# CognitiveAISystems/pogema

Hardware: AMD Instinct MI355X
Metric: agent-steps/sec (whole node), 64-agent 64x64 grid, batch=8192 envs (higher is better)
Workload: dtype u32

## Files before the change

include/pogema_amd.h:

```cpp
#ifndef POGEMA_AMD_H
#define POGEMA_AMD_H

#include <stddef.h>
#include <stdint.h>

#ifdef __cplusplus
extern "C" {
#endif

#define PGX_ABI_VERSION 6

#define PGX_OK 0
#define PGX_E_INVALID (-1)
#define PGX_E_HIP (-2)
#define PGX_E_NOMEM (-3)
#define PGX_E_STATE (-4)
#define PGX_E_PLACEMENT (-5)

#define PGX_COLLISION_PRIORITY 0
#define PGX_COLLISION_BLOCK_BOTH 1
#define PGX_COLLISION_SOFT 2

#define PGX_ON_TARGET_FINISH 0
#define PGX_ON_TARGET_RESTART 1
// ... 53 lines not shown

int pgx_create(const pgx_config* cfg, int device, pgx_env** out);
int pgx_destroy(pgx_env* env);
int pgx_check_config(const pgx_config* cfg);

int64_t pgx_obs_elems(const pgx_env* env);
int64_t pgx_agent_elems(const pgx_env* env);

int pgx_reset_from_state(pgx_env* env, const uint8_t* obstacles, const int32_t* agent_xy,
                         const int32_t* target_xy, void* stream);

int pgx_reset_random(pgx_env* env, float density, uint64_t seed, const uint8_t* shared_map,
                     const uint8_t* env_mask, int32_t max_retries, void* stream);

int pgx_regenerate(pgx_env* env, const uint8_t* env_mask, float density, uint64_t seed, const uint8_t* shared_map,
                   int32_t max_retries, void* obs, void* stream);
int64_t pgx_regenerate_failures(pgx_env* env, void* stream);

int pgx_set_map_pool(pgx_env* env, const uint8_t* maps, int32_t num_maps, int32_t* capacity_out, void* stream);
int pgx_reset_pool(pgx_env* env, uint64_t seed, const uint8_t* env_mask, int32_t max_retries, void* stream);
int pgx_regenerate_pool(pgx_env* env, const uint8_t* env_mask, uint64_t seed, int32_t max_retries, void* obs,
                        void* stream);
int pgx_get_map_index(pgx_env* env, int32_t* map_index, void* stream);

int pgx_get_map(pgx_env* env, uint8_t* obstacles, void* stream);

int pgx_step(pgx_env* env, const void* actions, int action_dtype, void* obs, float* rewards,
             uint8_t* terminated, uint8_t* truncated, uint8_t* is_active, void* stream);

int pgx_step_held(pgx_env* env, const void* actions, int action_dtype, void* obs, uint8_t* held, int32_t refresh,
                  float* rewards, uint8_t* terminated, uint8_t* truncated, uint8_t* is_active, void* stream);
int pgx_held_available(const pgx_env* env);

int pgx_xcd_shares(pgx_env* env, int32_t* shares);
int pgx_xcd_tune(pgx_env* env, void* obs, void* obs_alt, int32_t rounds, float* us_equal, float* us_tuned, void* stream);

typedef struct pgx_geometry {
    int32_t lanes_per_env;
    int32_t waves;
    int32_t envs_per_wave;
    int32_t multi_wave;
    int32_t p16;
    int32_t stagger;
    int32_t store_policy;
    int32_t state_stores;
    int32_t grid;
    int32_t lds_bytes;
    int32_t for_rollout;
    int32_t xcd_aware;
} pgx_geometry;
int pgx_get_geometry(const pgx_env* env, int32_t for_rollout, pgx_geometry* out);

typedef struct pgx_rollout_io {
    const void* actions;
    void* obs;
    float* rewards;
    uint8_t* terminated;
    uint8_t* truncated;
    uint8_t* is_active;
    uint8_t* episode_done;
    float* metrics;
    int32_t action_dtype;
    int32_t obs_slots;
    int64_t obs_slot_stride;
    uint64_t policy_seed;
    int64_t policy_step0;
// ... 197 lines not shown
```

pogema_amd/_lib.py:

```python
from __future__ import annotations

import ctypes as C
import os

_HERE = os.path.dirname(os.path.abspath(__file__))
LIB_PATH = os.environ.get("PGX_LIB") or os.path.join(_HERE, "libpogema_amd.so")

PGX_ABI_VERSION = 6

COLLISION_SYSTEMS = {"priority": 0, "block_both": 1, "soft": 2}
ON_TARGET = {"finish": 0, "restart": 1, "nothing": 2}
ACTION_DTYPES = {"int8": 0, "int32": 1, "int64": 2}
SOFT_VERTEX_RULES = {"lowest_index": 0, "all_stay": 1}
SOFT_OCCUPANCY = {"index_order": 0, "exact": 1}
COOP_REWARDS = {"all_solved": 0, "per_agent": 1}
BAD_ACTIONS = {"noop": 0, "flag": 1}
LIFELONG_RNGS = {"build": 0, "numpy": 1}
def _obs_dtypes():
    import torch
    return {torch.float32: 0, torch.uint8: 1, torch.bfloat16: 2, torch.float16: 3}


def obs_elem_bytes(dtype) -> int:
    import torch
# ... 36 lines not shown
PLAN_FIXED_PRIORITY = 1
MAX_WHCA_HORIZON = 31
SWAP_MAX_WALK = 2048
OUTCOMES = ("STAY", "MOVED", "OBSTACLE", "SWAP", "OCCUPIED", "FOLLOW", "CONTESTED")
NUM_OUTCOMES = len(OUTCOMES)
POLICY_CHANNELS = {"obstacles": 0, "agents": 1, "target": 2, "other_goals": 3, "up": 4, "down": 5, "left": 6, "right": 7}
NUM_CHANNELS = len(POLICY_CHANNELS)
COPY_NO_CACHE = 1
DEFAULT_POLICY_CHANNELS = ("obstacles", "agents", "target", "up", "down", "left", "right")
GLOBAL_CHANNELS = {"obstacles": 0, "agents": 1, "targets": 2, "agent_ids": 3, "target_ids": 4}
NUM_GLOBAL_CHANNELS = len(GLOBAL_CHANNELS)
DEFAULT_GLOBAL_CHANNELS = ("obstacles", "agents", "targets")
GLOBAL_ID_CHANNELS = ("agent_ids", "target_ids")
GLOBAL_ID_MAX = {1: 255, 2: 256}
GLOBAL_BAND_CELLS = 8192
TOKEN_CLIP = 20
TOKEN_BLOCKED = 41
TOKEN_ACTION_NONE = 42
TOKEN_ACTION0 = 43
TOKEN_GREEDY0 = 48
TOKEN_PAD = 64
NUM_TOKENS = 65
TOKEN_HISTORY = 5
TOKEN_SLOT_LEN = 10
MAX_TOKEN_SLOTS = 32
MAX_TOKEN_LENGTH = 2048
TOKENS = {"CLIP": TOKEN_CLIP, "BLOCKED": TOKEN_BLOCKED, "ACTION_NONE": TOKEN_ACTION_NONE, "ACTION0": TOKEN_ACTION0,
          "GREEDY0": TOKEN_GREEDY0, "PAD": TOKEN_PAD, "NUM_TOKENS": NUM_TOKENS, "HISTORY": TOKEN_HISTORY,
          "SLOT_LEN": TOKEN_SLOT_LEN, "MAX_SLOTS": MAX_TOKEN_SLOTS, "MAX_LENGTH": MAX_TOKEN_LENGTH}


EXPORTED_SYMBOLS = (
    "pgx_abi_version", "pgx_last_error", "pgx_create", "pgx_check_config", "pgx_destroy", "pgx_obs_elems", "pgx_agent_elems",
    "pgx_reset_from_state", "pgx_reset_random", "pgx_regenerate", "pgx_regenerate_failures", "pgx_get_map", "pgx_step", "pgx_step_held", "pgx_held_available", "pgx_observe", "pgx_set_metrics_buffers", "pgx_get_state", "pgx_generate", "pgx_place_agents",
    "pgx_snapshot_bytes", "pgx_save_snapshot", "pgx_load_snapshot", "pgx_time_observe", "pgx_bad_action_count",
    "pgx_buffers_create", "pgx_buffers_ptr", "pgx_buffers_get_info", "pgx_buffers_destroy", "pgx_set_targets",
    "pgx_np_streams", "pgx_np_streams_host", "pgx_np_generate", "pgx_np_generate_host", "pgx_rollout", "pgx_buffers_stride", "pgx_buffers_drop", "pgx_xcd_shares", "pgx_xcd_tune", "pgx_buffers_create_at", "pgx_time_observe_pair", "pgx_buffers_va_reserved", "pgx_get_geometry",
    "pgx_expert_actions", "pgx_set_map_pool", "pgx_reset_pool", "pgx_regenerate_pool", "pgx_get_map_index",
    "pgx_cost_to_go", "pgx_cost_to_go_bytes", "pgx_cost_to_go_builds", "pgx_visible_agents", "pgx_pibt_actions",
    "pgx_goal_directions", "pgx_shield_actions", "pgx_pibt_plan", "pgx_move_outcomes",
    "pgx_policy_input", "pgx_copy_envs", "pgx_global_state", "pgx_global_state_check",
    "pgx_agent_tokens", "pgx_agent_tokens_length", "pgx_goal_paths", "pgx_pibt_swap_actions", "pgx_pibt_swap_plan",
    "pgx_agent_forecasts", "pgx_blocking", "pgx_path_conflicts", "pgx_whca_plan", "pgx_repair_plan",
)


class PgxError(RuntimeError):
    def __init__(self, code: int, message: str):
        super().__init__(f"pogema_amd engine error {code}: {message}")
        self.code = code


class PgxBuffersInfo(C.Structure):
    _fields_ = [("bytes", C.c_int64), ("count", C.c_int32), ("spread", C.c_int32), ("candidates", C.c_int32),
                ("reserved0", C.c_int32), ("same_zone_us", C.c_float), ("final_us", C.c_float), ("spacer_gib", C.c_double),
                ("buffer_gbs", C.c_float), ("reserved1", C.c_float)]


class PgxGeometry(C.Structure):
    _fields_ = [(n, C.c_int32) for n in ("lanes_per_env", "waves", "envs_per_wave", "multi_wave", "p16", "stagger",
                                          "store_policy", "state_stores", "grid", "lds_bytes", "for_rollout", "xcd_aware")]


class PgxRolloutIO(C.Structure):
    _fields_ = [("actions", C.c_void_p), ("obs", C.c_void_p), ("rewards", C.c_void_p), ("terminated", C.c_void_p),
                ("truncated", C.c_void_p), ("is_active", C.c_void_p), ("episode_done", C.c_void_p), ("metrics", C.c_void_p),
                ("action_dtype", C.c_int32), ("obs_slots", C.c_int32), ("obs_slot_stride", C.c_int64),
# ... 119 lines not shown
    lib.pgx_agent_forecasts.argtypes = [vp, i32, i32, i32, vp, vp, vp]
    lib.pgx_agent_forecasts.restype = C.c_int
    lib.pgx_blocking.argtypes = [vp, i32, i32, vp, vp, vp]
    lib.pgx_blocking.restype = C.c_int
    lib.pgx_path_conflicts.argtypes = [vp, vp, i32, i32, i32, vp, vp, vp, vp, vp]
    lib.pgx_path_conflicts.restype = C.c_int
    lib.pgx_copy_envs.argtypes = [vp, vp, vp, i32, i32, vp]
    lib.pgx_copy_envs.restype = C.c_int
    lib.pgx_set_map_pool.argtypes = [vp, vp, i32, vp, vp]
    lib.pgx_set_map_pool.restype = C.c_int
    lib.pgx_reset_pool.argtypes = [vp, u64, vp, i32, vp]
    lib.pgx_reset_pool.restype = C.c_int
    lib.pgx_regenerate_pool.argtypes = [vp, vp, u64, i32, vp, vp]
    lib.pgx_regenerate_pool.restype = C.c_int
    lib.pgx_get_map_index.argtypes = [vp, vp, vp]
    lib.pgx_get_map_index.restype = C.c_int
    lib.pgx_set_targets.argtypes = [vp, vp, vp, vp]
    lib.pgx_set_targets.restype = C.c_int
    lib.pgx_bad_action_count.argtypes = [vp, vp]
    lib.pgx_bad_action_count.restype = i64
    lib.pgx_time_observe.argtypes = [vp, vp, i32, C.POINTER(C.c_float), vp]
    lib.pgx_time_observe.restype = C.c_int
    lib.pgx_time_observe_pair.argtypes = [vp, vp, vp, i32, C.POINTER(C.c_float), vp]
    lib.pgx_time_observe_pair.restype = C.c_int
    lib.pgx_snapshot_bytes.argtypes = [vp]
    lib.pgx_snapshot_bytes.restype = i64
    lib.pgx_save_snapshot.argtypes = [vp, vp, vp]
    lib.pgx_load_snapshot.argtypes = [vp, vp, vp]
    lib.pgx_save_snapshot.restype = lib.pgx_load_snapshot.restype = C.c_int
    lib.pgx_step.argtypes = [vp, vp, C.c_int, vp, vp, vp, vp, vp, vp]
    lib.pgx_step_held.argtypes = [vp, vp, C.c_int, vp, vp, i32, vp, vp, vp, vp, vp]
    lib.pgx_held_available.argtypes = [vp]
    lib.pgx_step_held.restype = lib.pgx_held_available.restype = C.c_int
    lib.pgx_observe.argtypes = [vp, vp, vp]
    lib.pgx_set_metrics_buffers.argtypes = [vp, vp, vp]
    lib.pgx_get_state.argtypes = [vp, vp, vp, vp, vp, vp, vp]
    lib.pgx_generate.argtypes = [i32, i32, i32, i32, f32, u64, i64, i32, i32, vp, vp, vp]
    lib.pgx_place_agents.argtypes = [i32, i32, i32, i32, u64, i64, i32, i32, vp, i32, vp, vp]
    for name in ("pgx_create", "pgx_destroy", "pgx_reset_from_state", "pgx_reset_random", "pgx_regenerate", "pgx_get_map",
                 "pgx_step", "pgx_observe", "pgx_set_metrics_buffers", "pgx_set_metrics_buffers",
                 "pgx_get_state", "pgx_generate", "pgx_place_agents"):
        getattr(lib, name).restype = C.c_int
    if lib.pgx_abi_version() != PGX_ABI_VERSION:
        raise ImportError(f"{LIB_PATH}: ABI version {lib.pgx_abi_version()} != expected {PGX_ABI_VERSION}; rebuild")
    _lib = lib
    return lib


def check(status: int) -> None:
    if status != 0:
        msg = load().pgx_last_error()
        raise PgxError(status, msg.decode("utf-8", "replace") if msg else "unknown error")
```

pogema_amd/buffers.py:

```python
from __future__ import annotations

import atexit
import collections
import contextlib
import ctypes as C
import os
import threading

import numpy as np
import torch

from . import _lib

_TYPESTR = {torch.float32: "<f4", torch.uint8: "|u1", torch.float16: "<f2", torch.bfloat16: "<f2"}


class _Owner:

    def __init__(self, lib, handle):
        self._lib, self._handle = lib, handle

    def __del__(self):
        try:
            if self._handle is not None and self._handle.value:
# ... 284 lines not shown
            cdata = master.untyped_storage()._cdata
            base = hook(cdata)
            alias = master.detach()
            one = hook(cdata)
            view = alias[2:4].view(torch.int16)
            two = hook(cdata)
            del alias
            still = hook(cdata)
            del view
            back = hook(cdata)
            if not (one == base + 1 and two == base + 2 and still == base + 1 and back == base):
                why = f"torch._C._storage_Use_Count no longer counts tensors per storage ({base}, {one}, {two}, {still}, {back})"
        except Exception as exc:
            why = f"torch._C._storage_Use_Count self-test raised {exc!r}"
    if why is not None:
        import warnings
        warnings.warn(f"pogema_amd: {why} in torch {torch.__version__}; reuse_buffers='recycle' falls back to allocating "
                      f"fresh output tensors per step", RuntimeWarning, stacklevel=2)
        hook = None
    _HOOK = hook
    return hook


_UNSET = object()
_HOOK = _UNSET


class RecyclingOutputs:

    @staticmethod
    def available() -> bool:
        return storage_count_hook() is not None

    def __init__(self, obs_tensors, batch: int, agents: int, zone_ptrs=()):
        if not self.available():
            raise RuntimeError("torch._C._storage_Use_Count is missing or changed its meaning in this torch build")
        self._count = storage_count_hook()
        self._zone_ptrs = frozenset(int(p) for p in zone_ptrs)
        dev = obs_tensors[0].device
        n = batch * agents
        self._sets = []
        for obs in obs_tensors:
            block = torch.empty(n * 7 + 16, dtype=torch.uint8, device=dev)
            members = (obs, block[:4 * n].view(torch.float32).view(batch, agents),
                       block[4 * n:5 * n].view(torch.bool).view(batch, agents),
                       block[5 * n:6 * n].view(torch.bool).view(batch, agents),
                       block[6 * n:7 * n].view(torch.bool).view(batch, agents))
            storages = (obs.untyped_storage(), block.untyped_storage())
            self._sets.append((members, storages, tuple(st._cdata for st in storages)))
        del obs, block, members, storages
        self._idle = [tuple(self._count(c) for c in cdata) for _, _, cdata in self._sets]
        self._held = [torch.full((batch, agents), 255, dtype=torch.uint8, device=dev) for _ in self._sets]
        self._vouched = [None] * len(self._sets)
        self._next = 0
        self.taken = 0
        self.misses = 0

    def __len__(self):
        return len(self._sets)

    def obs_pointers(self):
        return [members[0].data_ptr() for members, _, _ in self._sets]

    def _is_idle(self, i: int) -> bool:
        cdata, idle = self._sets[i][2], self._idle[i]
        return self._count(cdata[0]) == idle[0] and self._count(cdata[1]) == idle[1]

    def free_sets(self) -> int:
        return sum(self._is_idle(i) for i in range(len(self._sets)))

    def retire(self):
        idle = [i for i in range(len(self._sets)) if self._is_idle(i)]
        out = [self._sets[i][0][0] for i in idle if self._sets[i][0][0].data_ptr() in self._zone_ptrs]
        for i in reversed(idle):
            del self._sets[i]
            del self._idle[i]
            del self._held[i]
            del self._vouched[i]
        self._next = 0
        return out

    def _take_index(self):
        n = len(self._sets)
        for k in range(n):
            i = (self._next + k) % n
            if self._is_idle(i):
                self._next = (i + 1) % n
                self.taken += 1
                return i
        self.misses += 1
        return None

    def _hand_out(self, i: int, with_obs: bool):
        m = self._sets[i][0]
        return (m[0].detach() if with_obs else None, m[1].detach(), m[2].detach(), m[3].detach(), m[4].detach())

    @staticmethod
    def _version(t):
        try:
            return t._version
        except Exception:
            return None

    def take(self, with_obs: bool = True):
        i = self._take_index()
        if i is None:
            return None
        if with_obs:
            self._vouched[i] = None
        return self._hand_out(i, with_obs)

    def take_for_step(self, with_obs: bool = True):
        i = self._take_index()
        if i is None:
            return None
        trusted = False
        if with_obs:
            v = self._vouched[i]
            trusted = v is not None and self._version(self._sets[i][0][0]) == v
            self._vouched[i] = None
        return self._hand_out(i, with_obs), self._held[i], trusted, i

    def vouch(self, i: int):
        self._vouched[i] = self._version(self._sets[i][0][0])
```

pogema_amd/csrc/pgx_api.cpp:

```cpp
#include "../../include/pogema_amd.h"

#include <hip/hip_runtime.h>

#include <algorithm>
#include <cstdarg>
#include <cstdio>
#include <cstdlib>
#include <cstring>
#include <new>
#include <string>
#include <vector>

#include "pgx_internal.h"

namespace {
thread_local std::string g_err;
}

namespace pgx {
int fail_msg(int code, const char* fmt, ...) {
    char buf[512];
    va_list ap;
    va_start(ap, fmt);
    vsnprintf(buf, sizeof buf, fmt, ap);
// ... 883 lines not shown
    DeviceGuard guard;
    if (const int rc = enter(guard, e, "pgx_get_map", true)) return rc;
    PGX_HIP(hipMemcpyAsync(obstacles, e->map_u8, (size_t)e->cfg.batch * e->cfg.height * e->cfg.width,
                           hipMemcpyDeviceToDevice, (hipStream_t)stream));
    return PGX_OK;
}

int pgx_step(pgx_env* e, const void* actions, int action_dtype, void* obs, float* rewards, uint8_t* terminated,
             uint8_t* truncated, uint8_t* is_active, void* stream) {
    if (!e || !actions || !rewards || !terminated || !truncated) return fail_msg(PGX_E_INVALID, "pgx_step: null argument");
    if (const int rc = check_action_dtype("pgx_step", action_dtype)) return rc;
    DeviceGuard guard;
    if (const int rc = enter(guard, e, "pgx_step", true)) return rc;
    pgx::StepParams p = step_params(e, e->geo);
    p.mode = pgx::MODE_STEP;
    p.action_dtype = action_dtype;
    p.actions = actions;
    p.obs = static_cast<float*>(obs);
    p.rewards = rewards;
    p.terminated = terminated;
    p.truncated = truncated;
    p.act_out = is_active;
    PGX_HIP(pgx::launch_step(p, e->geo, (hipStream_t)stream));
    return PGX_OK;
}

int pgx_held_available(const pgx_env* e) {
    if (!e) return 0;
    return pgx::held_available(e->geo, e->cfg.num_agents, e->W, obs_elem_bytes(e->cfg.obs_dtype)) ? 1 : 0;
}

int pgx_step_held(pgx_env* e, const void* actions, int action_dtype, void* obs, uint8_t* held, int32_t refresh, float* rewards,
                  uint8_t* terminated, uint8_t* truncated, uint8_t* is_active, void* stream) {
    if (!e || !obs || !held || !pgx_held_available(e))
        return pgx_step(e, actions, action_dtype, obs, rewards, terminated, truncated, is_active, stream);
    if (!actions || !rewards || !terminated || !truncated) return fail_msg(PGX_E_INVALID, "pgx_step_held: null argument");
    if (const int rc = check_action_dtype("pgx_step_held", action_dtype)) return rc;
    DeviceGuard guard;
    if (const int rc = enter(guard, e, "pgx_step_held", true)) return rc;
    pgx::StepParams p = step_params(e, e->geo);
    p.mode = pgx::MODE_STEP;
    p.action_dtype = action_dtype;
    p.actions = actions;
    p.obs = static_cast<float*>(obs);
    p.rewards = rewards;
    p.terminated = terminated;
    p.truncated = truncated;
    p.act_out = is_active;
    PGX_HIP(pgx::launch_step_held(p, e->geo, held, refresh != 0, (hipStream_t)stream));
    return PGX_OK;
}

int pgx_rollout(pgx_env* e, int32_t steps, const pgx_rollout_io* io, void* stream) {
    if (!e || !io || !io->rewards || !io->terminated || !io->truncated)
        return fail_msg(PGX_E_INVALID, "pgx_rollout: null argument");
    if (io->policy_step0 < 0 || io->policy_step0 > ((int64_t)1 << 40))
        return fail_msg(PGX_E_INVALID, "pgx_rollout: policy_step0 outside 0..2^40");
    if (steps < 1) return fail_msg(PGX_E_INVALID, "pgx_rollout: steps must be >= 1, got %d", steps);
    if (const int rc = check_action_dtype("pgx_rollout", io->action_dtype)) return rc;
    if (io->obs && io->obs_slots < 1) return fail_msg(PGX_E_INVALID, "pgx_rollout: obs given but obs_slots = %d", io->obs_slots);
    DeviceGuard guard;
    if (const int rc = enter(guard, e, "pgx_rollout", true)) return rc;
    pgx::StepParams p = step_params(e, e->geo_roll);
    p.mode = pgx::MODE_STEP;
    p.action_dtype = io->action_dtype;
    p.actions = io->actions;
    p.obs = static_cast<float*>(io->obs);
    p.rewards = io->rewards;
    p.terminated = io->terminated;
    p.truncated = io->truncated;
    p.act_out = io->is_active;
    p.metrics_out = io->metrics;
    p.episode_done = io->episode_done;
    const int64_t agents = (int64_t)e->cfg.batch * e->cfg.num_agents;
    const int64_t W = 2 * e->cfg.obs_radius + 1;
    static const int64_t action_bytes[3] = {1, 4, 8};
    pgx::RolloutParams rp;
    rp.steps = steps;
    rp.obs_slots = io->obs ? io->obs_slots : 1;
    rp.resident_bitmap = e->geo_roll.resident_bitmap ? 1 : 0;
    rp.reserved0 = 0;
    rp.actions_stride = agents * action_bytes[io->action_dtype];
// ... 831 lines not shown
```

pogema_amd/csrc/pgx_internal.h:

```cpp
#pragma once
#include <hip/hip_runtime.h>
#include <stddef.h>
#include <stdint.h>

namespace pgx {

int fail_msg(int code, const char* fmt, ...);

#define PGX_HIP(call)                                                                                                      \
    do {                                                                                                                   \
        const hipError_t e__ = (call);                                                                                     \
        if (e__ != hipSuccess)                                                                                             \
            return pgx::fail_msg(PGX_E_HIP, "%s failed: %s (%s:%d)", #call, hipGetErrorString(e__), __FILE__, __LINE__); \
    } while (0)

struct DeviceGuard {
    int prev = -1;
    bool changed = false;
    hipError_t err = hipSuccess;
    DeviceGuard() = default;
    explicit DeviceGuard(int dev) { (void)select(dev); }
    DeviceGuard(const DeviceGuard&) = delete;
    DeviceGuard& operator=(const DeviceGuard&) = delete;
    hipError_t select(int dev) {
// ... 82 lines not shown
    int64_t env_index_base;
    const uint32_t* obst;
    uint32_t* pos;
    uint32_t* tgt;
    uint8_t* active;
    int32_t* elapsed;
    const uint32_t* pos0;
    const uint32_t* tgt0;
    const uint32_t* comp_begin;
    const uint32_t* comp_len;
    const uint32_t* comp_cells;
    uint32_t* tcount;
    NpGen* np_state;
    const NpGen* np_state0;
    int4* macc;
    float* metrics_out;
    uint8_t* episode_done;
    uint32_t* bad_count;
    const void* actions;
    float* obs;
    float* rewards;
    uint8_t* terminated;
    uint8_t* truncated;
    uint8_t* act_out;
    const uint8_t* only;
    unsigned long long* dbg;
};

struct HeldParams {
    uint8_t* held;
    int32_t refresh;
    int32_t lds_word;
    int32_t words;
};

struct RolloutParams {
    int32_t steps;
    int32_t obs_slots;
    int32_t resident_bitmap;
    int32_t reserved0;
    int64_t actions_stride;
    int64_t agents_stride;
    int64_t envs_stride;
    int64_t obs_stride;
    uint64_t policy_seed;
    int64_t policy_step0;
    int8_t* actions_out;
};

struct StepGeometry {
    int G;
    int waves;
    int epw;
    bool multi_wave;
    bool p16;
    int stagger;
    int store_policy;
    int state_stores;
    bool big;
    bool pc;
    bool resident_bitmap;
    size_t lds_bytes;
    int grid;
    int32_t xcd_n[8], xcd_base[8];
};
StepGeometry step_geometry(int batch, int A, int bmw, int W, bool allow_p16, int epw_override, int obs_elem_bytes,
                           int waves_override, bool for_rollout = false);
hipError_t prepare_step(const StepGeometry& g, const StepGeometry& roll);
hipError_t raise_lds_limit(const void* fn, size_t lds_bytes);
hipError_t launch_step(const StepParams& p, const StepGeometry& g, hipStream_t stream);
bool held_available(const StepGeometry& g, int A, int W, int obs_elem_bytes);
hipError_t prepare_step_held(const StepGeometry& g, int A, int W);
hipError_t launch_step_held(const StepParams& p, const StepGeometry& g, uint8_t* held, bool refresh, hipStream_t stream);
int xcd_partition(int blocks, const float w[8], int32_t n[8], int32_t base[8]);
hipError_t launch_rollout(const StepParams& p, const RolloutParams& rp, const StepGeometry& g, hipStream_t stream);

hipError_t launch_pack_obstacles(const uint8_t* obstacles, const uint8_t* only, uint32_t* bm, int batch, int H, int Wd,
                                 int r, int wpr, int bmw, const OutsideParams& outside, hipStream_t stream);

struct ResetParams {
    int32_t env_begin, env_count;
    int32_t H, Wd, A, r, wpr, bmw;
    int32_t lifelong;
    int32_t given_state;
    int32_t max_retries;
    uint32_t thr;
    uint64_t gen_seed;
    int64_t env_index_base;
    const uint8_t* shared_map;
    uint8_t* todo;
    const uint32_t* epoch;
    uint8_t* scratch_map;
    uint32_t* labels;
    uint32_t* pending;
    uint8_t* map_u8;
    uint32_t* obst_bm;
    uint32_t *pos, *tgt, *pos0, *tgt0;
    uint8_t* active;
    uint32_t* tcount;
    NpGen* np_state;
    const NpGen* np_state0;
    int32_t* elapsed;
    int4* macc;
    uint32_t *comp_begin, *comp_len, *comp_cells;
    uint32_t* fail_count;
    OutsideParams outside;
// ... 249 lines not shown
```

pogema_amd/csrc/pgx_kernels.hip:

```cpp
#include <hip/hip_runtime.h>
#include <stdint.h>
#include <stdlib.h>

#include <array>
#include <type_traits>
#include <map>
#include <mutex>
#include <string>
#include <vector>
#include <utility>

#include "pgx_internal.h"
#include "pgx_nprng.h"

namespace pgx {

__device__ __forceinline__ uint32_t lifelong_draw(uint64_t seed, uint64_t env_index, uint32_t agent,
                                                  uint32_t counter, uint32_t n) {
    uint64_t h = gen_sm64(seed);
    h = gen_sm64(h ^ env_index);
    h = gen_sm64(h ^ (((uint64_t)agent << 32) | counter));
    return (uint32_t)(((h >> 32) * (uint64_t)n) >> 32);
}

// ... 440 lines not shown
            macc = c.macc;
        }
        if (valid) {
            if (!given) {
                act = policy_action((uint64_t)rp.policy_seed, (uint64_t)(p.env_index_base + env), (uint32_t)agent,
                                    (uint64_t)(rp.policy_step0 + t));
                if (rp.actions_out) rp.actions_out[gi + (size_t)t * stride] = (int8_t)act;
            } else {
                act = (int)((c.ablk >> (4 * (t & 7))) & 15u);
                if ((t & 7) == 0 && t + 8 < steps) {
                    fetch_block = true;
#pragma unroll
                    for (int k = 0; k < 8; ++k) araw[k] = t + 8 + k < steps ? load_action(gi + (size_t)(t + 8 + k) * stride) : 0;
                }
            }
        }
      }
    } else {
    if (valid) {
        pos = p.pos[gi];
        tgt = p.tgt[gi];
        const uint32_t ab = p.active[gi];
        active = (ab & ACTIVE_BIT) != 0;
        ghost_in = (ab & ACTIVE_GHOST) != 0;
        if (p.mode == MODE_STEP) {
            if (p.action_dtype == 0) act = ((const int8_t*)p.actions)[gi];
            else if (p.action_dtype == 1) act = ((const int32_t*)p.actions)[gi];
            else act = (int)((const int64_t*)p.actions)[gi];
        }
    }
    if (env_ok && p.mode == MODE_STEP) elapsed = p.elapsed[env];
    env_leader = env_ok && agent == 0 && p.mode == MODE_STEP;
    if (env_leader) macc = p.macc[env];
    }

    if (do_resolve) {
        const uint32_t* g = p.obst + (size_t)env0 * bmw;
        const int n = nenv * bmw;
        const int stagger = (ROLL && t > 0) ? 0 : p.stagger;
        bool stage = true;
        if constexpr (ROLL) stage = t == 0 || !rp.resident_bitmap;
        if constexpr (BIG) stage = false;
        if (!stage) {
#pragma unroll 4
            for (int i = tid; i < n; i += NT) s_occ[i] = 0u;
        } else if (!MW && stagger > 0 && n <= 16 * 64) {
            uint32_t bmr[16];
#pragma unroll
            for (int k = 0; k < 16; ++k) bmr[k] = (tid + 64 * k < n) ? g[tid + 64 * k] : 0u;
            const uint32_t slot = __builtin_amdgcn_s_getreg(4 | (0 << 6) | (3 << 11));
            asm volatile("s_waitcnt vmcnt(0)" ::: "memory");
            if (slot & 1u)
                for (int k = 0; k < stagger; ++k) __builtin_amdgcn_s_sleep(127);
#pragma unroll
            for (int k = 0; k < 16; ++k)
                if (tid + 64 * k < n) {
                    s_obst[tid + 64 * k] = bmr[k];
                    s_occ[tid + 64 * k] = 0u;
                }
        } else
#pragma unroll 4
        for (int i = tid; i < n; i += NT) {
            s_obst[i] = g[i];
            s_occ[i] = 0u;
        }
        if (MW && tid < MISC_WORDS) s_misc[tid] = 0u;
// ... 323 lines not shown
                                }
                            }
    #pragma unroll
                            for (int k = 0; k < RB; ++k) {
                                const int wy = w8 + k;
                                if (wy < (WT ? WT : 16) && (WT || wy < W)) {
                                    const uint32_t bits = (uint32_t)((((uint64_t)hi[k] << 32) | lo[k]) >> sh) & wmask;
                                    rp[t][wy >> 1] |= bits << (16 * (wy & 1));
                                }
                            }
                            asm volatile("" ::: "memory");
                        }
                    }
                } else {
                    const uint32_t tc = s_atgt[la];
                    int dx = x - (int)(tc >> 16), dy = y - (int)(tc & 0xFFFFu);
                    dx = max(-r, min(r, dx));
                    dy = max(-r, min(r, dy));
                    const int hit = r - dx;
                    const uint32_t val = (1u << (r - dy)) << (16 * (hit & 1));
#pragma unroll
                    for (int m = 0; m < RW; ++m) rp[t][m] = (m == (hit >> 1)) ? val : 0u;
                }
            }
        }
        if constexpr (HELD) {
            if (tid < nag) {
                const int la = tid;
                const uint32_t cell = s_apos[la], tc = s_atgt[la];
                const int dx = max(-r, min(r, (int)(cell >> 16) - (int)(tc >> 16)));
                const int dy = max(-r, min(r, (int)(cell & 0xFFFFu) - (int)(tc & 0xFFFFu)));
                const uint32_t now = (uint32_t)((r - dx) * W + (r - dy));
                hp.held[(size_t)env0 * A + la] = (uint8_t)now;
                if (held_was < (uint32_t)(W * W)) {
                    constexpr int UL = PGX_HELD_UNIT_LOG2;
                    const uintptr_t slice = reinterpret_cast<uintptr_t>(obs_out + (size_t)env0 * A * 3 * W * W);
                    const uintptr_t plane = slice + (size_t)(la * 3 + 2) * (size_t)(W * W) * 4;
                    const uintptr_t ub = slice >> UL;
                    const int u1 = (int)(((plane + (size_t)(W * W) * 4) >> UL) - ub);
                    const int uw = (int)(((plane + held_was * 4) >> UL) - ub), un = (int)(((plane + now * 4) >> UL) - ub);
                    for (int u = (int)(((plane + ((1u << UL) - 1u)) >> UL) - ub); u < u1; ++u)
                        if (u != uw && u != un) atomicOr(&smem[hp.lds_word + (u >> 5)], 1u << (u & 31));
                }
            }
        }
        lds_sync<MW>();
        uint16_t* rows16 = reinterpret_cast<uint16_t*>(rows_base);
#pragma unroll
        for (int t = 0; t < 3; ++t) {
            const int item = tid + t * NT;
            if (item < nag * 3) {
#pragma unroll
                for (int wy = 0; wy < (WT ? WT : 16); ++wy)
                    if (WT || wy < W) rows16[item * W + wy] = (uint16_t)(rp[t][wy >> 1] >> (16 * (wy & 1)));
            }
        }
        if (tid < 4) rows16[nag * 3 * W + tid] = 0;
        lds_sync<MW>();

        const int n = nag * 3 * W * W;
        const size_t base = (size_t)env0 * A * 3 * W * W;
        if constexpr (WT == 0) {
        if (p.obs_one && W >= 7) {
            uint16_t* o = reinterpret_cast<uint16_t*>(obs_out) + base;
            const int head = min(n, (int)((8 - (base & 7)) & 7));
            const int nvec = (n - head) >> 3;
            const int tail0 = head + (nvec << 3);
            if (tid < 16) {
                const int e = (tid < 8) ? tid : tail0 + (tid - 8);
                if ((tid < 8) ? (tid < head) : (e < n)) {
                    const int row = (int)__umulhi((uint32_t)e, p.w_magic);
                    o[e] = (uint16_t)((((uint32_t)rows16[row] >> (e - row * W)) & 1u) * p.obs_one);
                }
            }
            const bool span = MW && !(p.flags & 512u);
            const int part = (nvec + nw - 1) / nw;
            const int q0 = span ? wave * part + lane : tid, q1 = span ? min(nvec, (wave + 1) * part) : nvec;
            const int e0 = head + (q0 << 3);
            const int row0 = (int)__umulhi((uint32_t)e0, p.w_magic);
// ... 499 lines not shown
        int upto = x == 7 ? blocks : (int)(acc * blocks + 0.5);
        if (upto > blocks) upto = blocks;
        if (upto < given) upto = given;
        n[x] = upto - given;
        base[x] = given;
        given = upto;
        if (n[x] > grid) grid = n[x];
    }
    return grid * 8;
}

static const void* held_fn_for(const StepGeometry& g) {
    if (g.big || !g.p16) return nullptr;
    if (g.multi_wave) return reinterpret_cast<const void*>(&step_held<64, true>);
#define PGX_CASE(gg) case gg: return reinterpret_cast<const void*>(&step_held<gg, false>);
    switch (g.G) {
        PGX_CASE(1) PGX_CASE(2) PGX_CASE(4) PGX_CASE(8) PGX_CASE(16) PGX_CASE(32) PGX_CASE(64)
        default: return nullptr;
    }
#undef PGX_CASE
}

static int held_words(size_t slice_bytes) {
    const size_t units = (slice_bytes >> PGX_HELD_UNIT_LOG2) + 2;
    return (int)(units / 32 + 1);
}

bool held_available(const StepGeometry& g, int A, int W, int obs_elem_bytes) {
    if (!held_fn_for(g) || obs_elem_bytes != 4 || W > 15) return false;
    const size_t slice = (size_t)g.epw * A * 3 * W * W * 4;
    return g.lds_bytes + (size_t)held_words(slice) * 4 <= 160 * 1024;
}

hipError_t prepare_step_held(const StepGeometry& g, int A, int W) {
    const size_t slice = (size_t)g.epw * A * 3 * W * W * 4;
    return raise_lds_limit(held_fn_for(g), g.lds_bytes + (size_t)held_words(slice) * 4);
}

hipError_t launch_step_held(const StepParams& p, const StepGeometry& g, uint8_t* held, bool refresh, hipStream_t stream) {
    const void* fn = held_fn_for(g);
    if (!fn) return hipErrorInvalidValue;
    StepParams args = p;
    HeldParams h;
    const int W = 2 * p.r + 1;
    h.held = held;
    h.refresh = refresh ? 1 : 0;
    h.lds_word = (int32_t)(g.lds_bytes / 4);
    h.words = held_words((size_t)g.epw * p.num_agents * 3 * W * W * 4);
    void* kargs[] = {&args, &h};
    return hipLaunchKernel(fn, dim3(g.grid), dim3(64 * g.waves), kargs, g.lds_bytes + (size_t)h.words * 4, stream);
}

hipError_t launch_step(const StepParams& p, const StepGeometry& g, hipStream_t stream) {
    const void* fn = step_fn_for(g);
    if (!fn) return hipErrorInvalidValue;
    StepParams args = p;
    void* kargs[] = {&args};
    return hipLaunchKernel(fn, dim3(g.grid), dim3(64 * g.waves), kargs, g.lds_bytes, stream);
}


hipError_t launch_pack_obstacles(const uint8_t* obstacles, const uint8_t* only, uint32_t* bm, int batch, int H, int Wd,
                                 int r, int wpr, int bmw, const OutsideParams& outside, hipStream_t stream) {
    const size_t total = (size_t)batch * bmw;
    const int bs = 256;
    hipLaunchKernelGGL(pack_obstacles_kernel, dim3((unsigned)((total + bs - 1) / bs)), dim3(bs), 0, stream,
                       obstacles, only, bm, batch, H, Wd, r, wpr, bmw, outside);
    return hipGetLastError();
}

hipError_t launch_pack_agents(const int32_t* agent_xy, const int32_t* target_xy, uint32_t* pos, uint32_t* tgt,
                              uint32_t* pos0, uint32_t* tgt0, uint8_t* active, uint32_t* tcount, size_t n,
                              int r, hipStream_t stream, NpGen* np_state, const NpGen* np_state0) {
    const int bs = 256;
    hipLaunchKernelGGL(pack_agents_kernel, dim3((unsigned)((n + bs - 1) / bs)), dim3(bs), 0, stream, agent_xy,
                       target_xy, pos, tgt, pos0, tgt0, active, tcount, n, r, np_state, np_state0);
    return hipGetLastError();
}

hipError_t launch_init_np_lifelong(NpGen* np_state0, uint64_t seed, int64_t env_index_base, int batch, int A, hipStream_t stream) {
    hipLaunchKernelGGL(init_np_lifelong_kernel, dim3((batch + 63) / 64), dim3(64), 0, stream, np_state0, seed, env_index_base, batch, A);
// ... 34 lines not shown
```

pogema_amd/placement.py:

```python
from __future__ import annotations

import ctypes as C
import os
from typing import Optional

import numpy as np
import torch

from . import _lib


def choose_buffers(zone_us, plain_us, n, margin=0.98):
    chosen = [("zone", i) for i in range(min(n, len(zone_us)))]
    time_of = {"zone": zone_us, "torch": plain_us}
    for j, t in enumerate(plain_us):
        if len(chosen) < n:
            chosen.append(("torch", j))
            continue
        worst = max(chosen, key=lambda c: time_of[c[0]][c[1]])
        if t < margin * time_of[worst[0]][worst[1]]:
            chosen[chosen.index(worst)] = ("torch", j)
    return chosen


# ... 169 lines not shown
        if probe:
            self.placement.update(probe)
        if fallback is not None:
            self.placement["fallback"] = fallback
            torch.cuda.empty_cache()
        bufs = [torch.empty(self.obs_shape, dtype=self.obs_dtype, device=self.device) for _ in range(n)]
        if self.placement_probe and self.batch >= 2048:
            self.placement.update(self.tune_xcd_shares(bufs[0], bufs[-1] if n > 1 else None))
        return bufs

    @staticmethod
    def _recycle_sets(obs_bytes: int) -> int:
        return 2 if (64 << 20) <= obs_bytes < (256 << 20) else 3

    def _build_recycler(self):
        from .buffers import RecyclingOutputs
        if not RecyclingOutputs.available():
            return False
        obs_bytes = int(np.prod(self.obs_shape)) * _lib.obs_elem_bytes(self.obs_dtype)
        n = self._recycle_sets(obs_bytes)
        if not self.placement_probe or obs_bytes < self.PLACEMENT_MIN_BYTES:
            bufs = self._plain_obs_buffers(n)
        else:
            from .buffers import ParkedBuffers
            parked = ParkedBuffers.claim(self._shelf_key(), n)
            if parked is not None:
                bufs, info = parked
                self._zone_ptrs = {t.data_ptr() for t in bufs}
                self.placement = dict(info, method="pgx_buffers (two HBM zones per buffer; taken over from a closed environment)")
                if self.batch >= 2048:
                    self.placement.update(self.tune_xcd_shares(bufs[0], bufs[-1] if n > 1 else None))
            else:
                bufs = self._pick_obs_buffers(n)
        return RecyclingOutputs(bufs, self.batch, self.num_agents, zone_ptrs=self._zone_ptrs)

    def tune_xcd_shares(self, obs: torch.Tensor, obs_alt: Optional[torch.Tensor] = None, rounds: int = 6) -> dict:
        if not self._has_state():
            return {}
        eq, tuned = C.c_float(0.0), C.c_float(0.0)
        _lib.check(self._lib.pgx_xcd_tune(self._handle, obs.data_ptr(), obs_alt.data_ptr() if obs_alt is not None else None,
                                          int(rounds), C.byref(eq), C.byref(tuned), self._stream()))
        shares = (C.c_int32 * 8)()
        _lib.check(self._lib.pgx_xcd_shares(self._handle, shares))
        return {"xcd_shares": list(shares), "observe_us_equal_shares": round(eq.value, 1), "observe_us_tuned_shares": round(tuned.value, 1)}

    PLAIN_CANDIDATES = 8

    SPARE_BUFFERS = 4

    def _time_observe(self, obs: torch.Tensor, obs_alt: Optional[torch.Tensor] = None) -> float:
        if not self._has_state():
            return 0.0
        us = C.c_float(0.0)
        if obs_alt is not None:
            _lib.check(self._lib.pgx_time_observe_pair(self._handle, obs.data_ptr(), obs_alt.data_ptr(), 8, C.byref(us), self._stream()))
            return float(us.value)
        _lib.check(self._lib.pgx_time_observe(self._handle, obs.data_ptr(), 3, C.byref(us), self._stream()))
        return float(us.value)

    def _ring_from_recycler(self, slots: int, obs_bytes: int):
        if not self.recycle or self._recycler is False:
            return None
        if self._recycler is None:
            if not self._has_state() or torch.cuda.is_current_stream_capturing():
                return None
            self._recycler = self._build_recycler()
        rec = self._recycler
# ... 90 lines not shown
```

pogema_amd/vec_env.py:

```python
from __future__ import annotations

import ctypes as C
import os
import warnings
from typing import Optional

import numpy as np
import torch

from . import _lib
from .grid_config import GridConfig
from .placement import PlacementMixin, choose_buffers
from .queries import QueryMixin
from .semantics import Semantics


def _as_device_index(device) -> int:
    dev = torch.device(device)
    if dev.type != "cuda":
        raise ValueError(f"VecPogema runs on a HIP device only, got {device!r}")
    return dev.index if dev.index is not None else torch.cuda.current_device()


def parse_map_pool(maps) -> torch.Tensor:
# ... 561 lines not shown
        if actions.dtype not in (torch.int8, torch.int32, torch.int64):
            actions = actions.to(torch.int64)
        if actions.numel() != self.batch * self.num_agents:
            raise ValueError(f"expected {self.batch}x{self.num_agents} actions, got shape {tuple(actions.shape)}")
        return actions.contiguous()

    _ACTION_CODE = {torch.int8: 0, torch.int32: 1, torch.int64: 2}

    def _check_out(self, out):
        if len(out) != 5:
            raise ValueError("out must be (obs, rewards, terminated, truncated, is_active)")
        B, A = self.batch, self.num_agents
        want = ((self.obs_shape, self.obs_dtype), ((B, A), torch.float32), ((B, A), torch.bool), ((B, A), torch.bool),
                ((B, A), torch.bool))
        for name, t, (shape, dtype) in zip(("obs", "rewards", "terminated", "truncated", "is_active"), out, want):
            if t is None and name == "obs":
                continue
            ok_dtype = t.dtype == dtype or (dtype == torch.bool and t.dtype == torch.uint8)
            if tuple(t.shape) != tuple(shape) or not ok_dtype or not t.is_contiguous() or t.device != self.device:
                raise ValueError(f"out[{name}] must be a contiguous {dtype} tensor of shape {tuple(shape)} on {self.device}")
        return out

    def step(self, actions, compute_obs: bool = True, out=None):
        actions = self._prepare_actions(actions)
        if out is not None:
            obs, rewards, terminated, truncated, is_active = self._check_out(out)
            if compute_obs and obs is None:
                raise ValueError("out[obs] is None but compute_obs=True")
        else:
            held = self._held_outputs(compute_obs) if self._held_on else None
            if held is not None:
                (obs, rewards, terminated, truncated, is_active), record, trusted, index = held
                if compute_obs:
                    _lib.check(self._lib.pgx_step_held(
                        self._handle, actions.data_ptr(), self._ACTION_CODE[actions.dtype], obs.data_ptr(), record.data_ptr(),
                        0 if trusted else 1, rewards.data_ptr(), terminated.data_ptr(), truncated.data_ptr(),
                        is_active.data_ptr(), self._stream()))
                    self._recycler.vouch(index)
                    self._held_steps += 1
                    self._held_refreshes += 0 if trusted else 1
                    infos = {"is_active": is_active, "episode_done": self.episode_done, "metrics": self.metrics}
                    if self.semantics.bad_action == "flag":
                        self._raise_on_bad_actions()
                    return self._wrap_obs(obs), rewards, terminated, truncated, infos
            elif self._held_on and self._recycler and not torch.cuda.is_current_stream_capturing():
                obs, rewards, terminated, truncated, is_active = self._alloc_outputs(compute_obs)
            else:
                obs, rewards, terminated, truncated, is_active = self._outputs(compute_obs)
        _lib.check(self._lib.pgx_step(
            self._handle, actions.data_ptr(), self._ACTION_CODE[actions.dtype],
            obs.data_ptr() if compute_obs else None, rewards.data_ptr(), terminated.data_ptr(),
            truncated.data_ptr(), is_active.data_ptr(), self._stream()))
        if self.regenerate:
            if self._reset_seed is None:
                raise RuntimeError("auto_reset='regenerate' needs reset(seed) first (random instances)")
            if self._pool is not None:
                _lib.check(self._lib.pgx_regenerate_pool(
                    self._handle, self.episode_done.data_ptr(), self._reset_seed, 3,
                    obs.data_ptr() if compute_obs else None, self._stream()))
            else:
                if self._shared is None and self.grid_config.map is not None:
                    self._shared = self._shared_map_tensor()
                _lib.check(self._lib.pgx_regenerate(
                    self._handle, self.episode_done.data_ptr(), float(self.grid_config.density), self._reset_seed,
                    self._shared.data_ptr() if self._shared is not None else None, 3,
                    obs.data_ptr() if compute_obs else None, self._stream()))
        if self.semantics.bad_action == "flag":
            self._raise_on_bad_actions()
        infos = {"is_active": is_active, "episode_done": self.episode_done, "metrics": self.metrics}
        return (self._wrap_obs(obs) if compute_obs else None), rewards, terminated, truncated, infos

    def _raise_on_bad_actions(self):
        bad = int(self._lib.pgx_bad_action_count(self._handle, self._stream()))
        if bad < 0:
            _lib.check(bad)
        if bad:
            raise IndexError(f"{bad} action(s) of active agents were outside 0..{len(self.grid_config.MOVES) - 1}")

    def _held_outputs(self, with_obs: bool):
        capturing = torch.cuda.is_current_stream_capturing()
        if self._recycler is None and self._has_state() and not capturing:
            self._recycler = self._build_recycler()
        if not self._recycler or capturing:
            return None
        return self._recycler.take_for_step(with_obs)

    def rollout(self, actions=None, obs_slots: Optional[int] = None, steps: Optional[int] = None, policy_seed: int = 0,
                policy_step0: int = 0, record_actions: bool = True):
        if self.regenerate:
            raise NotImplementedError("rollout() cannot draw new instances between its steps (auto_reset='regenerate')")
        if actions is None:
            if steps is None or int(steps) < 1:
                raise ValueError("rollout(actions=None) needs steps >= 1")
            K = int(steps)
        else:
            if not isinstance(actions, torch.Tensor):
                actions = torch.as_tensor(np.asarray(actions))
            if actions.dim() != 3 or tuple(actions.shape[1:]) != (self.batch, self.num_agents) or actions.shape[0] < 1:
                raise ValueError(f"actions must have shape [K >= 1, {self.batch}, {self.num_agents}], got {tuple(actions.shape)}")
            if steps is not None and int(steps) != int(actions.shape[0]):
                raise ValueError("steps does not match actions.shape[0]")
            if actions.dtype not in self._ACTION_CODE:
                actions = actions.to(torch.int64)
            actions = actions.to(self.device).contiguous()
            K = int(actions.shape[0])
        slots = K if obs_slots is None else int(obs_slots)
        if slots < 0:
            raise ValueError("obs_slots must be >= 0")
        slots = min(slots, K)
        dev, BA = self.device, (K, self.batch, self.num_agents)
# ... 117 lines not shown
```

Measured before the change: 5.203 billion.

## Track written observation lines per held buffer to skip rewriting unchanged regions

Adds a per-buffer bitmask of which observation cache-line units were written on the last use of each recycled output buffer. The held step kernel builds this mask in LDS with atomicOr over the agent-plane rows that hold nonzero data. It combines the new mask with the mask from the previous step so that only stale lines need clearing, replacing the per-agent clearing that used the held position. The aim is to cut redundant global stores of obs zeros. In exchange the kernel does extra LDS atomics, a global load and store of the line mask, and more register pressure.

```diff
diff --git a/include/pogema_amd.h b/include/pogema_amd.h
--- a/include/pogema_amd.h
+++ b/include/pogema_amd.h
@@ -109,6 +109,11 @@
                   float* rewards, uint8_t* terminated, uint8_t* truncated, uint8_t* is_active, void* stream);
 int pgx_held_available(const pgx_env* env);
 
+int pgx_step_held_lines(pgx_env* env, const void* actions, int action_dtype, void* obs, uint8_t* held, uint32_t* lines,
+                        int32_t refresh, float* rewards, uint8_t* terminated, uint8_t* truncated, uint8_t* is_active,
+                        void* stream);
+int64_t pgx_held_lines_words(const pgx_env* env);
+
 int pgx_xcd_shares(pgx_env* env, int32_t* shares);
 int pgx_xcd_tune(pgx_env* env, void* obs, void* obs_alt, int32_t rounds, float* us_equal, float* us_tuned, void* stream);
 
diff --git a/pogema_amd/_lib.py b/pogema_amd/_lib.py
--- a/pogema_amd/_lib.py
+++ b/pogema_amd/_lib.py
@@ -92,7 +92,7 @@
 
 EXPORTED_SYMBOLS = (
     "pgx_abi_version", "pgx_last_error", "pgx_create", "pgx_check_config", "pgx_destroy", "pgx_obs_elems", "pgx_agent_elems",
-    "pgx_reset_from_state", "pgx_reset_random", "pgx_regenerate", "pgx_regenerate_failures", "pgx_get_map", "pgx_step", "pgx_step_held", "pgx_held_available", "pgx_observe", "pgx_set_metrics_buffers", "pgx_get_state", "pgx_generate", "pgx_place_agents",
+    "pgx_reset_from_state", "pgx_reset_random", "pgx_regenerate", "pgx_regenerate_failures", "pgx_get_map", "pgx_step", "pgx_step_held", "pgx_held_available", "pgx_step_held_lines", "pgx_held_lines_words", "pgx_observe", "pgx_set_metrics_buffers", "pgx_get_state", "pgx_generate", "pgx_place_agents",
     "pgx_snapshot_bytes", "pgx_save_snapshot", "pgx_load_snapshot", "pgx_time_observe", "pgx_bad_action_count",
     "pgx_buffers_create", "pgx_buffers_ptr", "pgx_buffers_get_info", "pgx_buffers_destroy", "pgx_set_targets",
     "pgx_np_streams", "pgx_np_streams_host", "pgx_np_generate", "pgx_np_generate_host", "pgx_rollout", "pgx_buffers_stride", "pgx_buffers_drop", "pgx_xcd_shares", "pgx_xcd_tune", "pgx_buffers_create_at", "pgx_time_observe_pair", "pgx_buffers_va_reserved", "pgx_get_geometry",
@@ -278,6 +278,10 @@
     lib.pgx_step_held.argtypes = [vp, vp, C.c_int, vp, vp, i32, vp, vp, vp, vp, vp]
     lib.pgx_held_available.argtypes = [vp]
     lib.pgx_step_held.restype = lib.pgx_held_available.restype = C.c_int
+    lib.pgx_step_held_lines.argtypes = [vp, vp, C.c_int, vp, vp, vp, i32, vp, vp, vp, vp, vp]
+    lib.pgx_step_held_lines.restype = C.c_int
+    lib.pgx_held_lines_words.argtypes = [vp]
+    lib.pgx_held_lines_words.restype = C.c_int64
     lib.pgx_observe.argtypes = [vp, vp, vp]
     lib.pgx_set_metrics_buffers.argtypes = [vp, vp, vp]
     lib.pgx_get_state.argtypes = [vp, vp, vp, vp, vp, vp, vp]
diff --git a/pogema_amd/buffers.py b/pogema_amd/buffers.py
--- a/pogema_amd/buffers.py
+++ b/pogema_amd/buffers.py
@@ -340,7 +340,7 @@
     def available() -> bool:
         return storage_count_hook() is not None
 
-    def __init__(self, obs_tensors, batch: int, agents: int, zone_ptrs=()):
+    def __init__(self, obs_tensors, batch: int, agents: int, zone_ptrs=(), line_words: int = 0):
         if not self.available():
             raise RuntimeError("torch._C._storage_Use_Count is missing or changed its meaning in this torch build")
         self._count = storage_count_hook()
@@ -359,6 +359,7 @@
         del obs, block, members, storages
         self._idle = [tuple(self._count(c) for c in cdata) for _, _, cdata in self._sets]
         self._held = [torch.full((batch, agents), 255, dtype=torch.uint8, device=dev) for _ in self._sets]
+        self._lines = [torch.zeros(int(line_words), dtype=torch.int32, device=dev) if line_words else None for _ in self._sets]
         self._vouched = [None] * len(self._sets)
         self._next = 0
         self.taken = 0
@@ -384,6 +385,7 @@
             del self._sets[i]
             del self._idle[i]
             del self._held[i]
+            del self._lines[i]
             del self._vouched[i]
         self._next = 0
         return out
@@ -429,5 +431,8 @@
             self._vouched[i] = None
         return self._hand_out(i, with_obs), self._held[i], trusted, i
 
+    def line_record(self, i: int):
+        return self._lines[i]
+
     def vouch(self, i: int):
         self._vouched[i] = self._version(self._sets[i][0][0])
diff --git a/pogema_amd/csrc/pgx_api.cpp b/pogema_amd/csrc/pgx_api.cpp
--- a/pogema_amd/csrc/pgx_api.cpp
+++ b/pogema_amd/csrc/pgx_api.cpp
@@ -939,6 +939,22 @@
 
 int pgx_step_held(pgx_env* e, const void* actions, int action_dtype, void* obs, uint8_t* held, int32_t refresh, float* rewards,
                   uint8_t* terminated, uint8_t* truncated, uint8_t* is_active, void* stream) {
+    return pgx_step_held_lines(e, actions, action_dtype, obs, held, nullptr, refresh, rewards, terminated, truncated, is_active, stream);
+}
+
+static int lines_slice_words(const pgx_env* e) {
+    return pgx::held_lines_slice_words(e->geo, e->cfg.num_agents, e->W, obs_elem_bytes(e->cfg.obs_dtype));
+}
+
+int64_t pgx_held_lines_words(const pgx_env* e) {
+    if (!e) return 0;
+    const int64_t slices = e->geo.multi_wave ? e->cfg.batch : (e->cfg.batch + e->geo.epw - 1) / e->geo.epw;
+    return slices * lines_slice_words(e);
+}
+
+int pgx_step_held_lines(pgx_env* e, const void* actions, int action_dtype, void* obs, uint8_t* held, uint32_t* lines,
+                        int32_t refresh, float* rewards, uint8_t* terminated, uint8_t* truncated, uint8_t* is_active,
+                        void* stream) {
     if (!e || !obs || !held || !pgx_held_available(e))
         return pgx_step(e, actions, action_dtype, obs, rewards, terminated, truncated, is_active, stream);
     if (!actions || !rewards || !terminated || !truncated) return fail_msg(PGX_E_INVALID, "pgx_step_held: null argument");
@@ -954,7 +970,8 @@
     p.terminated = terminated;
     p.truncated = truncated;
     p.act_out = is_active;
-    PGX_HIP(pgx::launch_step_held(p, e->geo, held, refresh != 0, (hipStream_t)stream));
+    if (!lines_slice_words(e)) lines = nullptr;
+    PGX_HIP(pgx::launch_step_held(p, e->geo, held, lines, refresh != 0, (hipStream_t)stream));
     return PGX_OK;
 }
 
diff --git a/pogema_amd/csrc/pgx_internal.h b/pogema_amd/csrc/pgx_internal.h
--- a/pogema_amd/csrc/pgx_internal.h
+++ b/pogema_amd/csrc/pgx_internal.h
@@ -138,6 +138,7 @@
     int32_t refresh;
     int32_t lds_word;
     int32_t words;
+    uint32_t* lines;
 };
 
 struct RolloutParams {
@@ -177,7 +178,9 @@
 hipError_t launch_step(const StepParams& p, const StepGeometry& g, hipStream_t stream);
 bool held_available(const StepGeometry& g, int A, int W, int obs_elem_bytes);
 hipError_t prepare_step_held(const StepGeometry& g, int A, int W);
-hipError_t launch_step_held(const StepParams& p, const StepGeometry& g, uint8_t* held, bool refresh, hipStream_t stream);
+int held_lines_slice_words(const StepGeometry& g, int A, int W, int obs_elem_bytes);
+hipError_t launch_step_held(const StepParams& p, const StepGeometry& g, uint8_t* held, uint32_t* lines, bool refresh,
+                            hipStream_t stream);
 int xcd_partition(int blocks, const float w[8], int32_t n[8], int32_t base[8]);
 hipError_t launch_rollout(const StepParams& p, const RolloutParams& rp, const StepGeometry& g, hipStream_t stream);
 
diff --git a/pogema_amd/csrc/pgx_kernels.hip b/pogema_amd/csrc/pgx_kernels.hip
--- a/pogema_amd/csrc/pgx_kernels.hip
+++ b/pogema_amd/csrc/pgx_kernels.hip
@@ -496,6 +496,10 @@
     if (env_ok && p.mode == MODE_STEP) elapsed = p.elapsed[env];
     env_leader = env_ok && agent == 0 && p.mode == MODE_STEP;
     if (env_leader) macc = p.macc[env];
+    }
+    [[maybe_unused]] uint32_t lines_old = 0u;
+    if constexpr (HELD) {
+        if (hp.lines && !hp.refresh && tid < hp.words) lines_old = hp.lines[(size_t)blk * hp.words + tid];
     }
 
     if (do_resolve) {
@@ -885,7 +889,7 @@
                 const int dy = max(-r, min(r, (int)(cell & 0xFFFFu) - (int)(tc & 0xFFFFu)));
                 const uint32_t now = (uint32_t)((r - dx) * W + (r - dy));
                 hp.held[(size_t)env0 * A + la] = (uint8_t)now;
-                if (held_was < (uint32_t)(W * W)) {
+                if (!hp.lines && held_was < (uint32_t)(W * W)) {
                     constexpr int UL = PGX_HELD_UNIT_LOG2;
                     const uintptr_t slice = reinterpret_cast<uintptr_t>(obs_out + (size_t)env0 * A * 3 * W * W);
                     const uintptr_t plane = slice + (size_t)(la * 3 + 2) * (size_t)(W * W) * 4;
@@ -897,7 +901,50 @@
                 }
             }
         }
+        [[maybe_unused]] const uintptr_t slice_addr = reinterpret_cast<uintptr_t>(obs_out + (size_t)env0 * A * 3 * W * W);
+        if constexpr (HELD) {
+            if (hp.lines) {
+                constexpr int UL = PGX_HELD_UNIT_LOG2;
+                const uint32_t soff = (uint32_t)(slice_addr & ((1u << UL) - 1u));
+#pragma unroll
+                for (int t = 0; t < 3; ++t) {
+                    const int item = tid + t * NT;
+                    if (item < nag * 3) {
+                        const uint32_t pbyte = soff + (uint32_t)item * (uint32_t)(W * W * 4);
+                        const uint32_t u0 = pbyte >> UL, pb = pbyte & ((1u << UL) - 1u);
+                        uint32_t lm = 0u;
+#pragma unroll
+                        for (int wy = 0; wy < (WT ? WT : 16); ++wy) {
+                            const uint32_t m = (rp[t][wy >> 1] >> (16 * (wy & 1))) & 0xFFFFu;
+                            if ((WT || wy < W) && m) {
+                                const uint32_t f = pb + (uint32_t)(wy * W * 4);
+                                lm |= 1u << ((f + 4u * (uint32_t)__builtin_ctz(m)) >> UL);
+                                lm |= 1u << ((f + 4u * (31u - (uint32_t)__builtin_clz(m))) >> UL);
+                            }
+                        }
+                        const uint64_t wide = (uint64_t)lm << (u0 & 31u);
+                        if ((uint32_t)wide) atomicOr(&smem[hp.lds_word + (u0 >> 5)], (uint32_t)wide);
+                        if ((uint32_t)(wide >> 32)) atomicOr(&smem[hp.lds_word + (u0 >> 5) + 1], (uint32_t)(wide >> 32));
+                    }
+                }
+            }
+        }
         lds_sync<MW>();
+        if constexpr (HELD) {
+            if (hp.lines && tid < hp.words) {
+                constexpr int UL = PGX_HELD_UNIT_LOG2;
+                const int nfl = nag * 3 * W * W;
+                const uintptr_t lo = (slice_addr + 15u) & ~(uintptr_t)15u;
+                const uintptr_t hi = lo + (((uintptr_t)nfl * 4u - (lo - slice_addr)) & ~(uintptr_t)15u);
+                const int uf = (int)(((lo + ((1u << UL) - 1u)) >> UL) - (slice_addr >> UL));
+                const int ul = (int)((hi >> UL) - (slice_addr >> UL));
+                const int b0 = max(0, min(32, uf - 32 * tid)), b1 = max(0, min(32, ul - 32 * tid));
+                const uint32_t inside = b1 > b0 ? (uint32_t)((((uint64_t)1 << b1) - 1u) & ~(((uint64_t)1 << b0) - 1u)) : 0u;
+                const uint32_t rec = ~smem[hp.lds_word + tid] & inside;
+                smem[hp.lds_word + tid] = rec & lines_old;
+                hp.lines[(size_t)blk * hp.words + tid] = rec;
+            }
+        }
         uint16_t* rows16 = reinterpret_cast<uint16_t*>(rows_base);
 #pragma unroll
         for (int t = 0; t < 3; ++t) {
@@ -1463,12 +1510,19 @@
     return g.lds_bytes + (size_t)held_words(slice) * 4 <= 160 * 1024;
 }
 
+int held_lines_slice_words(const StepGeometry& g, int A, int W, int obs_elem_bytes) {
+    if (!held_available(g, A, W, obs_elem_bytes)) return 0;
+    const int words = held_words((size_t)g.epw * A * 3 * W * W * 4);
+    return words <= 64 * g.waves ? words : 0;
+}
+
 hipError_t prepare_step_held(const StepGeometry& g, int A, int W) {
     const size_t slice = (size_t)g.epw * A * 3 * W * W * 4;
     return raise_lds_limit(held_fn_for(g), g.lds_bytes + (size_t)held_words(slice) * 4);
 }
 
-hipError_t launch_step_held(const StepParams& p, const StepGeometry& g, uint8_t* held, bool refresh, hipStream_t stream) {
+hipError_t launch_step_held(const StepParams& p, const StepGeometry& g, uint8_t* held, uint32_t* lines, bool refresh,
+                            hipStream_t stream) {
     const void* fn = held_fn_for(g);
     if (!fn) return hipErrorInvalidValue;
     StepParams args = p;
@@ -1478,6 +1532,7 @@
     h.refresh = refresh ? 1 : 0;
     h.lds_word = (int32_t)(g.lds_bytes / 4);
     h.words = held_words((size_t)g.epw * p.num_agents * 3 * W * W * 4);
+    h.lines = lines;
     void* kargs[] = {&args, &h};
     return hipLaunchKernel(fn, dim3(g.grid), dim3(64 * g.waves), kargs, g.lds_bytes + (size_t)h.words * 4, stream);
 }
diff --git a/pogema_amd/placement.py b/pogema_amd/placement.py
--- a/pogema_amd/placement.py
+++ b/pogema_amd/placement.py
@@ -225,7 +225,8 @@
                     self.placement.update(self.tune_xcd_shares(bufs[0], bufs[-1] if n > 1 else None))
             else:
                 bufs = self._pick_obs_buffers(n)
-        return RecyclingOutputs(bufs, self.batch, self.num_agents, zone_ptrs=self._zone_ptrs)
+        return RecyclingOutputs(bufs, self.batch, self.num_agents, zone_ptrs=self._zone_ptrs,
+                                line_words=self._held_line_words())
 
     def tune_xcd_shares(self, obs: torch.Tensor, obs_alt: Optional[torch.Tensor] = None, rounds: int = 6) -> dict:
         if not self._has_state():
diff --git a/pogema_amd/vec_env.py b/pogema_amd/vec_env.py
--- a/pogema_amd/vec_env.py
+++ b/pogema_amd/vec_env.py
@@ -617,10 +617,11 @@
             if held is not None:
                 (obs, rewards, terminated, truncated, is_active), record, trusted, index = held
                 if compute_obs:
-                    _lib.check(self._lib.pgx_step_held(
+                    lines = self._recycler.line_record(index)
+                    _lib.check(self._lib.pgx_step_held_lines(
                         self._handle, actions.data_ptr(), self._ACTION_CODE[actions.dtype], obs.data_ptr(), record.data_ptr(),
-                        0 if trusted else 1, rewards.data_ptr(), terminated.data_ptr(), truncated.data_ptr(),
-                        is_active.data_ptr(), self._stream()))
+                        lines.data_ptr() if lines is not None else None, 0 if trusted else 1, rewards.data_ptr(),
+                        terminated.data_ptr(), truncated.data_ptr(), is_active.data_ptr(), self._stream()))
                     self._recycler.vouch(index)
                     self._held_steps += 1
                     self._held_refreshes += 0 if trusted else 1
@@ -661,6 +662,9 @@
             _lib.check(bad)
         if bad:
             raise IndexError(f"{bad} action(s) of active agents were outside 0..{len(self.grid_config.MOVES) - 1}")
+
+    def _held_line_words(self) -> int:
+        return int(self._lib.pgx_held_lines_words(self._handle)) if self._held_on else 0
 
     def _held_outputs(self, with_obs: bool):
         capturing = torch.cuda.is_current_stream_capturing()
```

Result: no change. 5.249 billion (median of 5 runs) (+0.9%).
